# jscanvic/Scale-Equivariant-Imaging

Hardware: AMD Instinct MI355X
Metric: training images/sec (256x256 crops), proposed-loss deblur (higher is better)
Workload: dtype bf16; 1 GPU; BASELINE configs[1]: deblurring Gaussian_R2 noise=5, proposed loss (SURE + scale-EI), 256x256 pairs cropped to 48 in Loss.forward, ConvolutionalModel hidden=32 scales=5; parameters=645063043, batch_per_gpu=32, global_batch=32, parallelism=dp1

## Files before the change

### include/sei_hip.h

```cpp
#ifndef SEI_HIP_H
#define SEI_HIP_H

#include <stddef.h>
#include <stdint.h>

#ifdef __cplusplus
extern "C" {
#endif

#define SEI_OK 0
#define SEI_ERR_BAD_ARG 10001
#define SEI_ERR_TOO_LARGE 10002


#define SEI_ABI_VERSION 12
int sei_abi_version(void);
int sei_build_target(char *name, int n);

int sei_event_create(void **event);
int sei_event_destroy(void *event);
int sei_event_record_external(void *event, void *stream);
int sei_stream_wait_event(void *stream, void *event);

int sei_graph_node_counts(void *graph, int *kernel_nodes, int *all_nodes);
// ... 380 lines not shown
int sei_dwstream_bf16_jobs(const SeiDwStreamJob *jobs, int njobs, void *stream);
size_t sei_dwstream_bf16_eligible(int Mo, int Ni, int ldy, int ldx, long long K1, long long K2);

int sei_rowgemm_bf16(const uint16_t *A, int lda, const uint16_t *W, int ldw, float *D32, int ld32, uint16_t *D16,
                     int ld16, long long M, int N, int K, int nv, int epilogue, const float *bias, const float *R1,
                     const float *R2, int ldr, void *stream);
size_t sei_rowgemm_bf16_eligible(long long M, int N, int K, int epilogue, int out16);

int sei_rowgemm_lnbwd_bf16(const uint16_t *A, int lda, const uint16_t *W, int ldw, long long M, int K, const float *x,
                           const float *gamma, const float *mean, const float *rstd, const float *res, float *gx, int C,
                           float *ggamma, float *gbeta, const float *row_scale, uint16_t *y16, int ldy, float *colsum,
                           float *work, size_t work_floats, void *stream);
size_t sei_rowgemm_lnbwd_bf16_eligible(long long M, int K, int C);
size_t sei_rowgemm_lnbwd_work_floats(int C);

int sei_rowgemm_dgelu_bf16(const uint16_t *A, int lda, const uint16_t *W, int ldw, const uint16_t *A2, int lda2,
                           const uint16_t *W2, int ldw2, const float *bias2, int nv, uint16_t *D16, int ld16, long long M,
                           int N, int K, void *stream);
size_t sei_rowgemm_dgelu_bf16_eligible(long long M, int N, int K);

int sei_rowgemm_ln_bf16(const uint16_t *A, int lda, const uint16_t *W, int ldw, long long M, int K, int C, const float *bias,
                        const float *row_scale, const float *res, float *out, const float *gamma, const float *beta,
                        float eps, int ones_col, uint16_t *h16, int ldh, float *mean, float *rstd, void *stream);
size_t sei_rowgemm_ln_bf16_eligible(long long M, int K, int C);

int sei_rowgemm_gelu_bf16(const uint16_t *A, int lda, const uint16_t *W, int ldw, const float *bias, int nv, uint16_t *D16,
                          int ld16, long long M, int N, int K, int one_at, void *stream);

size_t sei_drunet_work_bytes(int B, int H, int W);
int sei_drunet_conv3x3(const uint16_t *X, const uint16_t *Wt, int Cin, int Cout, int B, int H, int W, int epilogue,
// ... 67 lines not shown
```

### scale-equivariant-imaging_amd/_native.py

```python
import ctypes
import os

import torch

_HERE = os.path.dirname(os.path.abspath(__file__))
LIB_PATH = os.environ.get("SEI_HIP_LIBRARY") or os.path.join(_HERE, "libsei_hip.so")

SEI_REDUCE_BLOCKS = 256

_c = ctypes
_P, _I, _F, _Z, _L = _c.c_void_p, _c.c_int, _c.c_float, _c.c_size_t, _c.c_longlong

SIGNATURES = {
    "sei_abi_version": [],
    "sei_event_create": [_P],
    "sei_event_destroy": [_P],
    "sei_event_record_external": [_P, _P],
    "sei_stream_wait_event": [_P, _P],
    "sei_graph_node_counts": [_P, _P, _P],
    "sei_build_target": [_c.c_char_p, _I],
    "sei_blur_sep_circ": [_P, _P, _P, _P, _I, _I, _I, _I, _I, _I, _P],
    "sei_blur_dense_circ": [_P, _P, _P, _I, _I, _I, _I, _I, _I, _P],
    "sei_blur_dense_pad": [_P, _P, _P, _I, _I, _I, _I, _I, _I, _I, _P, _P],
    "sei_circ_filter_sep": [_P, _P, _P, _P, _I, _I, _I, _P],
# ... 98 lines not shown
    "sei_swin_attn_bwd_bf16": [_P, _P, _P, _P, _P, _P, _P, _I, _I, _I, _I, _I, _F, _P],
    "sei_pad_nhwc": [_P, _P, _I, _I, _I, _I, _I, _P],
    "sei_unpad_nhwc": [_P, _P, _P, _I, _I, _I, _I, _I, _P],
    "sei_rowscale": [_P, _P, _P, _P, _Z, _I, _P],
    "sei_pack": [_P, _P, _P, _Z, _I, _P],
    "sei_unpack_add": [_P, _P, _P, _Z, _P],
    "sei_ln_fwd_bf16_pad": [_P, _P, _P, _P, _P, _P, _Z, _I, _I, _F, _I, _P],
    "sei_ln_bwd_pad": [_P, _P, _P, _P, _P, _P, _P, _P, _P, _Z, _I, _I, _P, _Z, _P],
    "sei_cast_pad_bf16": [_P, _P, _P, _P, _Z, _I, _I, _P, _Z, _P],
    "sei_pad_nhwc_bf16": [_P, _P, _I, _I, _I, _I, _I, _I, _P],
    "sei_pad_nhwc_bf16_ones": [_P, _P, _I, _I, _I, _I, _I, _I, _I, _P],
    "sei_gemm_bf16nt_conv": [_P, _I, _P, _P, _I, _P, _P, _I, _I, _I, _P, _P],
    "sei_gemm_bf16nt_conv_unpad": [_P, _I, _P, _P, _I, _P, _P, _I, _I, _I, _I, _P, _I, _P],
    "sei_rowgemm_bf16": [_P, _I, _P, _I, _P, _I, _P, _I, _L, _I, _I, _I, _I, _P, _P, _P, _I, _P],
    "sei_rowgemm_lnbwd_bf16": [_P, _I, _P, _I, _L, _I, _P, _P, _P, _P, _P, _P, _I, _P, _P, _P, _P, _I, _P, _P, _Z, _P],
    "sei_rowgemm_dgelu_bf16": [_P, _I, _P, _I, _P, _I, _P, _I, _P, _I, _P, _I, _L, _I, _I, _P],
    "sei_rowgemm_ln_bf16": [_P, _I, _P, _I, _L, _I, _I, _P, _P, _P, _P, _P, _P, _F, _I, _P, _I, _P, _P, _P],
    "sei_rowgemm_gelu_bf16": [_P, _I, _P, _I, _P, _I, _P, _I, _L, _I, _I, _I, _P],
    "sei_tokgrad_bf16_blocks": [_P, _I, _L, _L, _P],
    "sei_tokgrad_bf16": [_P, _P, _I, _P, _P, _I, _P, _I, _I, _I, _L, _L, _P],
    "sei_dwstream_bf16_jobs": [_P, _I, _P],
    "sei_adam_fused": [_P, _P, _I, _P, _P, _Z, _F, _F, _F, _F, _F, _I, _F, _P, _P],
    "sei_adam_scalars": [_F, _F, _F, _F, _F, _I, _P, _P],
    "sei_adam_scalars_to_device": [_F, _F, _F, _F, _F, _I, _P, _P],
    "sei_sgd_fused": [_P, _P, _P, _P, _Z, _Z, _F, _F, _P, _P, _I, _P],
    "sei_sgd_penalty_finish": [_P, _Z, _P, _P],
    "sei_adam_anchor_fused": [_P, _P, _P, _P, _P, _P, _Z, _Z, _F, _F, _F, _F, _F, _I, _F, _P, _P, _I, _P],
    "sei_drunet_conv3x3": [_P, _P, _I, _I, _I, _I, _I, _I, _P, _P, _P, _P, _P],
    "sei_drunet_conv3x3_ex": [_P, _P, _I, _I, _I, _I, _I, _I, _P, _P, _P, _P, _I, _P],
    "sei_drunet_down": [_P, _P, _I, _I, _I, _I, _I, _P, _P, _P],
# ... 80 lines not shown
    "sei_dwconv7_bwd_weight_workspace": [_I, _I, _I, _I],
    "sei_dwconv7_bwd_weight_workspace_ex": [_I, _I, _I, _I, _I],
    "sei_ln_bwd_workspace": [_Z, _I],
    "sei_dwconv7_ln_fwd_launches": [_I, _I, _I, _I],
    "sei_sepmap2_bf16_eligible": [_I, _I, _I, _I, _I, _I],
    "sei_sepmap2_bf16_pack_elems": [_I, _I, _I, _I],
    "sei_sepmap2_big_eligible": [_I, _I, _I, _I, _I, _I],
    "sei_sepmap2_big_pack_elems": [_I, _I, _I, _I],
    "sei_sepmap2_big_work_elems": [_I, _I, _I, _I, _I, _I],
    "sei_swin_partials_floats": [_I],
    "sei_tokgrad_bf16_eligible": [_I, _I, _I, _I, _L, _L],
    "sei_dwstream_bf16_eligible": [_I, _I, _I, _I, _L, _L],
    "sei_mlp_fused_eligible": [_L, _I],
    "sei_rowgemm_bf16_eligible": [_L, _I, _I, _I, _I],
    "sei_rowgemm_lnbwd_bf16_eligible": [_L, _I, _I],
    "sei_rowgemm_lnbwd_work_floats": [_I],
    "sei_ln_bwd_part_offset": [_Z, _I],
    "sei_ln_bwd_part_count": [_Z, _I],
    "sei_rowgemm_dgelu_bf16_eligible": [_L, _I, _I],
    "sei_rowgemm_ln_bf16_eligible": [_L, _I, _I],
    "sei_gemm_bf16nt_plan": [_I, _I, _I, _I, _I, _I, _I, _I],
    "sei_gemm_bf16nt_plan_ws": [_I, _I, _I, _I, _I, _I, _I, _I, _Z],
    "sei_gemm_bf16nt_dw2_adam_plan": [_I, _I, _I, _I, _I],
    "sei_gemm_bf16nt_dw2_adam_groupable": [_I, _I, _I, _I],
    "sei_conv3x3_bwd_weight_parts_count": [_I, _I, _I, _I, _I, _I, _I],
    "sei_sepmap2_small_eligible": [_I, _I, _I, _I, _I, _I],
    "sei_cast_bf16_colsum_parts_count": [_I, _I],
    "sei_sgd_partials": [_Z, _Z, _I],
    "sei_adam_anchor_partials": [_Z, _Z, _I],
    "sei_drunet_work_bytes": [_I, _I, _I],
# ... 169 lines not shown
```

### scale-equivariant-imaging_amd/csrc/token_gemm.hip

```cpp
#include "rm_image.h"

namespace {

constexpr int TG_NW = 8, TG_NT = 64 * TG_NW;
constexpr int TG_WCN = 4;
constexpr int TG_RB = 6, TG_CB = 3;
constexpr int TG_NPIECE = 48 / TG_NW;
constexpr int TG_STAGE = 6 * RM_IMG;
constexpr int TG_MAX_BLOCKS = SEI_TOKGRAD_MAX_BLOCKS;

struct TokGradArgs {
    SeiTokGradBlock blk[TG_MAX_BLOCKS];
    int nblk;
    int kt_seg, kt_total;
    int workers_per_xcd;
};

struct TgRange {
    int bsel, kt0, nt;
};
__device__ __forceinline__ TgRange tg_range(const TokGradArgs &g) {
    const int xcd = blockIdx.x & 7, slot = blockIdx.x >> 3;
    const int wslot = slot / g.nblk, bsel = slot - wslot * g.nblk;
    if (wslot >= g.workers_per_xcd) return {0, 0, 0};
// ... 151 lines not shown
    const unsigned short *A2 = nullptr, *W2 = nullptr;
    int lda2 = 0, ldw2 = 0;
    const float *beta2 = nullptr;
    float *mean_out = nullptr, *rstd_out = nullptr;
    float eps = 0.f;
    int ones_col = 0;
    int gelu_one_at = -1;
};

constexpr int RG_EPI_LNBWD = 100;
constexpr int RG_EPI_DGELU2 = 101;
constexpr int RG_EPI_RES_LN = 102;
constexpr int RG_EPI_SCALE_RES_LN = 103;
constexpr int RG_EPI_GELU16 = 104;

template <int KT, int NBT, int TR, int WN, int WR, int EPI, bool OUT16>
__global__ __launch_bounds__(RG_NT, (EPI == RG_EPI_GELU16 ? 4 : 1)) void rowgemm_kernel(RowGemmArgs g) {
    constexpr int WK = 8 / (WN * WR);
    static_assert(WN * WR * WK == 8 && (WK == 1 || WK == 2), "eight waves");
    constexpr int NB = (NBT + WN - 1) / WN;
    constexpr int NBX = NBT % WN;
    constexpr int RB = TR / WR / 16;
    constexpr int KS = 2 * KT / WK;
    static_assert(TR % (16 * WR) == 0 && (2 * KT) % WK == 0, "whole blocks per wave");
    constexpr int NP = 16 * NBT;
    constexpr int LDP = NP + 4;
    constexpr bool TWO = EPI == RG_EPI_DGELU2;
    constexpr int OPS = TWO ? 2 : 1;
    constexpr int STAGE = OPS * KT * TR * 128;
    constexpr int P = KT * TR / 8;
    constexpr int EMAX = (P + 7) / 8;
    constexpr int QR = NP / 4;
    constexpr bool LNB = EPI == RG_EPI_LNBWD;
    constexpr bool LNF = EPI == RG_EPI_RES_LN || EPI == RG_EPI_SCALE_RES_LN;
    constexpr bool LNX = LNB || LNF;
    static_assert(!LNX || (NBT == 12 && TR == 32), "the LayerNorm epilogues own 32 rows x 192 columns: 16 lanes per row");
    constexpr int GQ = (!LNX && (OUT16 || EPI == SEI_EPI_MUL_DGELU || TWO)) ? 2 : 1;
    constexpr bool GELU16 = EPI == RG_EPI_GELU16;
    static_assert(!GELU16 || (OUT16 && WK == 1 && NBX == 0), "bf16 output only; whole column blocks per wave, all of K");
    constexpr bool P16 = ((EPI == SEI_EPI_BIAS || EPI == SEI_EPI_NONE) && OUT16) || TWO || GELU16;
    constexpr int LDP16 = NP + 8;
    static_assert(!P16 || WK == 1, "the bf16 patch has nothing to add up");
    constexpr int IR = QR / GQ;
    constexpr int IPT = (TR * IR + RG_NT - 1) / RG_NT;
    constexpr bool RAGGED = TR * IR % RG_NT != 0;
    constexpr int QPT = IPT * GQ;
    static_assert(TR % 16 == 0 && QR % GQ == 0, "whole items");
    constexpr bool HAS_ROWS = EPI == SEI_EPI_BIAS_RES || EPI == SEI_EPI_BIAS_SCALE_RES || EPI == SEI_EPI_MUL_DGELU;
    constexpr bool HAS_BIAS = EPI == SEI_EPI_BIAS || EPI == SEI_EPI_BIAS_GELU || EPI == SEI_EPI_BIAS_RES ||
                              EPI == SEI_EPI_BIAS_SCALE_RES || LNF;
    constexpr int UNR = IPT > 3 ? (GQ == 2 ? 2 : 3) : IPT;
    constexpr int NAUX = LNF ? 3 + (EPI == RG_EPI_SCALE_RES_LN ? 1 : 0) : LNB ? 8 + (OUT16 ? 1 : 0)
                             : (HAS_ROWS ? QPT : 0) + (EPI == SEI_EPI_BIAS_SCALE_RES ? QPT : 0);
    constexpr int PATCH_ONE = (P16 ? TR * LDP16 * 2 : TR * LDP * 4 + 15) / 16 * 16;
    constexpr int AUX_BYTES = GELU16 ? 0 : (LNF ? 3 : 1) * NP * 4;
    constexpr bool PATCH2 = !GELU16 && 3 * STAGE + 2 * PATCH_ONE + AUX_BYTES <= 160 * 1024;
    __shared__ __attribute__((aligned(1024))) char smem[3 * STAGE + (PATCH2 ? 2 : 1) * PATCH_ONE + AUX_BYTES];
    float *const patch0 = reinterpret_cast<float *>(smem + 3 * STAGE);
    float *lbias = reinterpret_cast<float *>(smem + 3 * STAGE + (PATCH2 ? 2 : 1) * PATCH_ONE);
    float *lgam = lbias + NP, *lbet = lgam + NP;

    const int tid = threadIdx.x, lane = tid & 63;
    const int wave = __builtin_amdgcn_readfirstlane(tid >> 6);
    const int wn = wave % WN, wr = (wave / WN) % WR, wk = wave / (WN * WR);
    const int nbw = (NBX == 0 || wn < NBX) ? NB : NB - 1;
    const int nb0 = (NBX == 0 || wn < NBX) ? NB * wn : NB * NBX + (NB - 1) * (wn - NBX);
    const int l16 = lane & 15, lg = lane >> 4;
    const int G = gridDim.x, b = blockIdx.x;
    if (b >= g.tiles) return;
    const int nt = (g.tiles - b + G - 1) / G;

    bf16x8 wf[NB][KS];
#pragma unroll
    for (int nb = 0; nb < NB; ++nb)
#pragma unroll
        for (int s = 0; s < KS; ++s)
            wf[nb][s] = *reinterpret_cast<const bf16x8 *>(g.W + (size_t)(16 * (nb0 + min(nb, nbw - 1)) + l16) * g.ldw +
                                                          32 * (wk * KS + s) + 8 * lg);
    bf16x8 wf2[TWO ? NB : 1][TWO ? KS : 1];
    float bias2[TWO ? NB : 1];
    if constexpr (TWO) {
#pragma unroll
        for (int nb = 0; nb < NB; ++nb) {
#pragma unroll
            for (int s = 0; s < KS; ++s)
                wf2[nb][s] = *reinterpret_cast<const bf16x8 *>(g.W2 + (size_t)(16 * (nb0 + min(nb, nbw - 1)) + l16) * g.ldw2 +
                                                               32 * (wk * KS + s) + 8 * lg);
            const int c = 16 * (nb0 + min(nb, nbw - 1)) + l16;
            bias2[nb] = c < g.nv ? g.bias[c] : 0.f;
        }
#pragma unroll
// ... 16 lines not shown
#pragma unroll
        for (int nb = 0; nb < NB; ++nb) is_one[nb] = 16 * (nb0 + min(nb, nbw - 1)) + l16 == g.gelu_one_at;
    }
    if constexpr (P16 && (EPI == SEI_EPI_BIAS || GELU16)) {
#pragma unroll
        for (int nb = 0; nb < NB; ++nb) {
            const int c = 16 * (nb0 + min(nb, nbw - 1)) + l16;
            biasr[nb] = c < g.nv ? g.bias[c] : 0.f;
        }
#pragma unroll
        for (int nb = 0; nb < NB; ++nb) asm volatile("" : "+v"(biasr[nb]));
    }
    unsigned offa[EMAX];
#pragma unroll
    for (int e = 0; e < EMAX; ++e) {
        const int q = min(wave + 8 * e, P - 1), im = q / (TR / 8), p = q % (TR / 8);
        const int r = 8 * p + (lane >> 3);
        const int c = (lane & 7) ^ ((r >> 1) & 7);
        offa[e] = (unsigned)r * (unsigned)g.lda * 2u + 128u * im + 16u * c;
    }
    unsigned offa2[TWO ? EMAX : 1];
    if constexpr (TWO) {
#pragma unroll
        for (int e = 0; e < EMAX; ++e) {
            const int q = min(wave + 8 * e, P - 1), im = q / (TR / 8), p = q % (TR / 8);
            const int r = 8 * p + (lane >> 3);
            const int c = (lane & 7) ^ ((r >> 1) & 7);
            offa2[e] = (unsigned)r * (unsigned)g.lda2 * 2u + 128u * im + 16u * c;
        }
    }
// ... 33 lines not shown
            const float *rows = EPI == SEI_EPI_BIAS_SCALE_RES ? g.R2 : g.R1;
#pragma unroll
            for (int i = 0; i < QPT; ++i) {
                const size_t row = (size_t)tile * TR + quad_row(i);
                const int qc = quad_col(i);
                const float *src = rows + row * g.ldr + (qc < g.nv ? qc : 0);
                asm volatile("global_load_dwordx4 %0, %1, off" : "=v"(a[i]) : "v"(src) : "memory");
                if constexpr (EPI == SEI_EPI_BIAS_SCALE_RES) {
                    const float *ssrc = g.R1 + row;
                    asm volatile("global_load_dword %0, %1, off" : "=v"(sc[i]) : "v"(ssrc) : "memory");
                }
            }
        }
    };

    const int er = tid >> 4, el = tid & 15;
    const int nvq = g.nv >> 2;
    f32x4 lx[LNX ? 3 : 1], lr[LNB ? 3 : 1], ag[LNB ? 3 : 1], ab[LNB ? 3 : 1], ac[LNB ? 3 : 1];
    float lmu = 0.f, lrs = 0.f, lsc = 1.f;
    if constexpr (LNF) {
        for (int c = tid; c < NP; c += RG_NT) {
            lgam[c] = c < g.nv ? g.gamma[c] : 0.f;
            lbet[c] = c < g.nv ? g.beta2[c] : 0.f;
        }
    }
    if constexpr (LNB) {
        for (int c = tid; c < NP; c += RG_NT) lbias[c] = c < g.nv ? g.gamma[c] : 0.f;
#pragma unroll
        for (int k = 0; k < 3; ++k) ag[k] = ab[k] = ac[k] = f32x4{0.f, 0.f, 0.f, 0.f};
    }
    auto load_ln = [&](int t) {
        if constexpr (LNF) {
            const int tile = b + min(t, nt - 1) * G;
            const size_t row = (size_t)tile * TR + er;
            const float *rows = EPI == RG_EPI_SCALE_RES_LN ? g.R2 : g.R1;
#pragma unroll
            for (int k = 0; k < 3; ++k) {
                const float *xs = rows + row * g.ldr + 4 * min(el + 16 * k, nvq - 1);
                asm volatile("global_load_dwordx4 %0, %1, off" : "=v"(lx[k]) : "v"(xs) : "memory");
            }
            if constexpr (EPI == RG_EPI_SCALE_RES_LN) {
                const float *cs = g.R1 + row;
                asm volatile("global_load_dword %0, %1, off" : "=v"(lsc) : "v"(cs) : "memory");
            }
        }
        if constexpr (LNB) {
            const int tile = b + min(t, nt - 1) * G;
            const size_t row = (size_t)tile * TR + er;
#pragma unroll
            for (int k = 0; k < 3; ++k) {
                const int c = 4 * min(el + 16 * k, nvq - 1);
                const float *xs = g.R1 + row * g.ldr + c, *rs = g.R2 + row * g.ldr + c;
                asm volatile("global_load_dwordx4 %0, %1, off" : "=v"(lx[k]) : "v"(xs) : "memory");
                asm volatile("global_load_dwordx4 %0, %1, off" : "=v"(lr[k]) : "v"(rs) : "memory");
            }
            const float *ms = g.mean + row, *ss = g.rstd + row;
            asm volatile("global_load_dword %0, %1, off" : "=v"(lmu) : "v"(ms) : "memory");
            asm volatile("global_load_dword %0, %1, off" : "=v"(lrs) : "v"(ss) : "memory");
            if constexpr (OUT16) {
                const float *cs = g.scale + row;
                asm volatile("global_load_dword %0, %1, off" : "=v"(lsc) : "v"(cs) : "memory");
            }
        }
    };

    issue(0);
    issue(1);
    if (P % 8 != 0 && wave < P % 8) sei_wait_vmcnt<NDMA_HI>();
    else sei_wait_vmcnt<NDMA_LO>();
    sei_lds_barrier();

    for (int t = 0; t < nt; ++t) {
        float *const patch = PATCH2 ? reinterpret_cast<float *>(reinterpret_cast<char *>(patch0) + (t & 1) * PATCH_ONE) : patch0;
        load_aux(t, cur, curs);
        load_ln(t);
        __builtin_amdgcn_sched_barrier(0);
// ... 33 lines not shown
                        float v;
                        if constexpr (TWO) v = acc[0][nb][j] * sei_dgelu_bf16out(acc2[nb][j] + bias2[nb]);
                        else v = is_one[nb] ? 1.0f : sei_gelu_bf16out(acc[0][nb][j] + biasr[nb]);
                        const __bf16 h = (__bf16)v;
                        pw16[(16 * rb + j) * LDP16 + 16 * nb] = __builtin_bit_cast(unsigned short, h);
                    }
            }
        } else {
#pragma unroll
        for (int rb = 0; rb < RB; ++rb)
#pragma unroll
            for (int nb = 0; nb < NB; ++nb) acc[rb][nb] = f32x4{0.f, 0.f, 0.f, 0.f};
#pragma unroll
        for (int s = 0; s < KS; ++s) {
            const int sg = wk * KS + s;
            const char *img = st + (sg >> 1) * (TR * 128) + (wr * RB * 16 + l16) * 128 + (((4 * (sg & 1) + lg) ^ (l16 >> 1)) * 16);
#pragma unroll
            for (int rb = 0; rb < RB; ++rb) {
                const bf16x8 fa = *reinterpret_cast<const bf16x8 *>(img + rb * 16 * 128);
#pragma unroll
                for (int nb = 0; nb < NB; ++nb) {
                    if (NBX != 0 && nb == NB - 1 && nbw < NB) break;
                    acc[rb][nb] = __builtin_amdgcn_mfma_f32_16x16x32_bf16(fa, wf[nb][s], acc[rb][nb], 0, 0, 0);
                }
            }
        }
        }
        if (P % 8 != 0 && wave < P % 8) sei_wait_vmcnt<NAUX + NDMA_HI>();
        else sei_wait_vmcnt<NAUX + NDMA_LO>();
        if constexpr (P16 && !GELU16 && !TWO) {
            unsigned short *pw16 = reinterpret_cast<unsigned short *>(patch) + (wr * RB * 16 + 4 * lg) * LDP16 + 16 * nb0 + l16;
#pragma unroll
            for (int rb = 0; rb < RB; ++rb)
#pragma unroll
// ... 94 lines not shown
                } else if (qk == nvq && g.ones_col) {
                    y[0] = 1.0f;
                }
                uint2 h;
                h.x = sei_pack2_bf16(y[0], y[1]);
                h.y = sei_pack2_bf16(y[2], y[3]);
                *reinterpret_cast<uint2 *>(g.D16 + row * g.ld16 + 4 * qk) = h;
            }
        }
        if constexpr (LNB) {
            __builtin_amdgcn_sched_barrier(0);
            if (P % 8 != 0 && wave < P % 8) sei_wait_vmcnt<NDMA_HI>();
            else sei_wait_vmcnt<NDMA_LO>();
            __builtin_amdgcn_sched_barrier(0);
#pragma unroll
            for (int k = 0; k < 3; ++k) {
                asm volatile("" : "+v"(lx[k]));
                asm volatile("" : "+v"(lr[k]));
            }
            asm volatile("" : "+v"(lmu));
            asm volatile("" : "+v"(lrs));
            if constexpr (OUT16) asm volatile("" : "+v"(lsc));
            f32x4 gh[3], xh[3], tq[3];
            float s1 = 0.f, s2 = 0.f;
#pragma unroll
            for (int k = 0; k < 3; ++k) {
                const bool valid = el + 16 * k < nvq;
                gh[k] = *reinterpret_cast<const f32x4 *>(patch + er * LDP + 4 * (el + 16 * k));
                const f32x4 gm = *reinterpret_cast<const f32x4 *>(lbias + 4 * (el + 16 * k));
#pragma unroll
                for (int j = 0; j < 4; ++j) {
                    xh[k][j] = (lx[k][j] - lmu) * lrs;
                    tq[k][j] = gh[k][j] * gm[j];
                }
                if (valid) {
                    s1 += (tq[k][0] + tq[k][1]) + (tq[k][2] + tq[k][3]);
                    s2 += (tq[k][0] * xh[k][0] + tq[k][1] * xh[k][1]) + (tq[k][2] * xh[k][2] + tq[k][3] * xh[k][3]);
                    ag[k] += gh[k] * xh[k];
                    ab[k] += gh[k];
                }
            }
#pragma unroll
            for (int off = 8; off > 0; off >>= 1) {
                s1 += __shfl_xor(s1, off, 16);
                s2 += __shfl_xor(s2, off, 16);
            }
            const float invC = 1.0f / (float)g.nv;
            s1 *= invC;
            s2 *= invC;
            const size_t row = row0 + er;
#pragma unroll
            for (int k = 0; k < 3; ++k) {
                const int qk = el + 16 * k;
                const bool valid = qk < nvq;
                f32x4 o;
#pragma unroll
                for (int j = 0; j < 4; ++j) o[j] = lrs * (tq[k][j] - s1 - xh[k][j] * s2) + lr[k][j];
                if (valid) *reinterpret_cast<f32x4 *>(g.D32 + row * g.ld32 + 4 * qk) = o;
                if constexpr (OUT16) {
                    f32x4 ys;
#pragma unroll
                    for (int j = 0; j < 4; ++j) ys[j] = valid ? o[j] * lsc : 0.f;
                    if constexpr (KT != 9) ac[k] += ys;
                    uint2 h;
                    h.x = sei_pack2_bf16(ys[0], ys[1]);
                    h.y = sei_pack2_bf16(ys[2], ys[3]);
                    *reinterpret_cast<uint2 *>(g.D16 + row * g.ld16 + 4 * qk) = h;
                }
            }
        }
        if constexpr (P16) {
#pragma unroll
            for (int it = 0; it < IPT; ++it) {
                if (RAGGED && it == IPT - 1 && tid + RG_NT * it >= TR * IR) break;
                const int idx = tid + RG_NT * it, qr = idx / IR, qc = 8 * (idx % IR);
                const uint4 h = *reinterpret_cast<const uint4 *>(reinterpret_cast<const unsigned short *>(patch) + qr * LDP16 + qc);
                *reinterpret_cast<uint4 *>(g.D16 + (row0 + qr) * g.ld16 + qc) = h;
            }
        }
#pragma unroll UNR
        for (int it = 0; it < ((LNX || P16) ? 0 : IPT); ++it) {
            if (RAGGED && it == IPT - 1 && tid + RG_NT * it >= TR * IR) break;
            f32x4 v[GQ];
// ... 25 lines not shown
                h.x = sei_pack2_bf16(ge[0], ge[1]);
                h.y = sei_pack2_bf16(ge[2], ge[3]);
                *reinterpret_cast<uint2 *>(g.D16 + row * g.ld16 + qc) = h;
            } else if constexpr (GQ == 2) {
                uint4 h;
                h.x = sei_pack2_bf16(v[0][0], v[0][1]);
                h.y = sei_pack2_bf16(v[0][2], v[0][3]);
                h.z = sei_pack2_bf16(v[GQ - 1][0], v[GQ - 1][1]);
                h.w = sei_pack2_bf16(v[GQ - 1][2], v[GQ - 1][3]);
                *reinterpret_cast<uint4 *>(g.D16 + row * g.ld16 + qc) = h;
            }
        }
        if constexpr (!PATCH2) sei_lds_barrier();
    }
    sei_wait_vmcnt<0>();
    if constexpr (LNB) {
        static_assert(3 * STAGE >= 3 * 32 * 48 * 16, "the ring holds the partial sums");
        __builtin_amdgcn_s_barrier();
        f32x4 *red = reinterpret_cast<f32x4 *>(smem);
#pragma unroll
        for (int k = 0; k < 3; ++k) {
            red[(0 * 32 + er) * 48 + el + 16 * k] = ag[k];
            red[(1 * 32 + er) * 48 + el + 16 * k] = ab[k];
            red[(2 * 32 + er) * 48 + el + 16 * k] = ac[k];
        }
        __syncthreads();
        if (tid < 144) {
            const int sel = tid / 48, qk = tid - sel * 48;
            f32x4 a = f32x4{0.f, 0.f, 0.f, 0.f};
            for (int r = 0; r < 32; ++r) a += red[(sel * 32 + r) * 48 + qk];
            if (qk < nvq) *reinterpret_cast<f32x4 *>(g.part + ((size_t)b * 3 + sel) * g.nv + 4 * qk) = a;
        }
    }
}

template <int KT, int NBT, int TR, int WN, int WR, int EPI, bool OUT16>
int rg_launch(const RowGemmArgs &g, int M, hipStream_t s, int per_cu = 1) {
    RowGemmArgs a = g;
    a.tiles = M / TR;
    const int grid = a.tiles < 256 * per_cu ? a.tiles : 256 * per_cu;
    hipLaunchKernelGGL((rowgemm_kernel<KT, NBT, TR, WN, WR, EPI, OUT16>), dim3((unsigned)grid), dim3(RG_NT), 0, s, a);
    return sei_launch_status();
}

bool rg_operands_ok(const uint16_t *A, int lda, const uint16_t *W, int ldw, int K) {
    return A && W && lda >= K && ldw >= K && lda % 8 == 0 && ldw % 8 == 0 && (((uintptr_t)A | (uintptr_t)W) & 15) == 0 &&
           (unsigned long long)64 * (size_t)lda * 2 < (1ull << 32);
}
int rg_fill_operands(RowGemmArgs &g, const uint16_t *A, int lda, const uint16_t *W, int ldw, long long M, int K) {
    SEI_REQUIRE(M > 0 && M % 64 == 0 && M < (1ll << 31) && rg_operands_ok(A, lda, W, ldw, K));
    g.A = A; g.W = W; g.lda = lda; g.ldw = ldw;
    return SEI_OK;
}

bool tg_block_ok(const SeiTokGradBlock &b, long long K2) {
    if (!b.Y1 || !b.X1 || !b.D || (K2 && (!b.Y2 || !b.X2))) return false;
// ... 127 lines not shown
    if (y16) SEI_REQUIRE(ldy >= 192 && ldy % 4 == 0 && ((uintptr_t)y16 & 7) == 0);
    g.R1 = x; g.R2 = res; g.ldr = C;
    g.D32 = gx; g.D16 = y16; g.ld32 = C; g.ld16 = ldy; g.nv = C;
    g.mean = mean; g.rstd = rstd; g.gamma = gamma; g.scale = row_scale; g.part = work;
    hipStream_t s = (hipStream_t)stream;
    const int m = (int)M, groups = m / 32 < 256 ? m / 32 : 256;
    int rc;
    if (K == 384)
        rc = y16 ? rg_launch<6, 12, 32, 4, 1, RG_EPI_LNBWD, true>(g, m, s) : rg_launch<6, 12, 32, 4, 1, RG_EPI_LNBWD, false>(g, m, s);
    else
        rc = y16 ? rg_launch<9, 12, 32, 4, 1, RG_EPI_LNBWD, true>(g, m, s) : rg_launch<9, 12, 32, 4, 1, RG_EPI_LNBWD, false>(g, m, s);
    if (rc != 0 || !ggamma) return rc;
    return sei_fold_now(sei_fold_job(SEI_FOLD_SPLIT, work, groups, 3 * C, C, ggamma, gbeta, colsum), s);
}

extern "C" size_t sei_rowgemm_dgelu_bf16_eligible(long long M, int N, int K) {
    return (M > 0 && M % 64 == 0 && M < (1ll << 31) && N == 384 && K == 192) ? 1 : 0;
}

extern "C" int sei_rowgemm_dgelu_bf16(const uint16_t *A, int lda, const uint16_t *W, int ldw, const uint16_t *A2, int lda2,
                                      const uint16_t *W2, int ldw2, const float *bias2, int nv, uint16_t *D16, int ld16,
                                      long long M, int N, int K, void *stream) {
    RowGemmArgs g;
    SEI_REQUIRE(bias2 && D16 && sei_rowgemm_dgelu_bf16_eligible(M, N, K));
    SEI_REQUIRE(rg_fill_operands(g, A, lda, W, ldw, M, K) == SEI_OK && rg_operands_ok(A2, lda2, W2, ldw2, K));
    SEI_REQUIRE(((uintptr_t)D16 & 15) == 0 && nv > 0 && nv <= N && ld16 >= N && ld16 % 8 == 0);
    g.A2 = A2; g.W2 = W2; g.lda2 = lda2; g.ldw2 = ldw2;
    g.bias = bias2; g.D16 = D16; g.ld16 = ld16; g.nv = nv;
    return rg_launch<3, 24, 32, 8, 1, RG_EPI_DGELU2, true>(g, (int)M, (hipStream_t)stream);
}
// ... 38 lines not shown
```

### scale-equivariant-imaging_amd/models/_ops.py

```python
import os

import torch

import _native as N
from . import _mats, _wgrad
from ._gemm import (EPI_ACCUM, EPI_BIAS, EPI_BIAS_GELU, EPI_BIAS_RES, EPI_BIAS_ROWSCALE, EPI_MUL_DGELU, EPI_NONE,
                    SPLITK_COUNTER_BYTES, SPLITK_WS_MIB, SPLITK_WS_STREAMS, _SPLITK_WS, _gemm_call, _in_forward_mode,
                    compute_dtype_scope, gemm, gemm_mixed, gemm_nt16, gemm_x3, get_compute_dtype, joint_rows,
                    own_splitk_workspace, profile_gemms, release_splitk_workspace, reset_splitk_counters, set_compute_dtype,
                    splitk_workspace)
from ._joint import JointCtx, _NotJoint, joint_ctx, walk_backward
from ._shadow import (ShadowState, _new_plain_state, _transposed16, _transposed16_cached, plain_shadow_is_current,
                      refresh_plain_shadow, set_stale_masters, shadow, split_x2, weights_updated)
from ._wgrad import (_state_for, begin_step, colsum16_into, defer_fold, direct_bf16_launches, flush_weight_grads,
                     fused_adam_launches, merged_weight_grads, note_forward, register_gradient_range,
                     set_direct_bf16_grads, set_fused_adam, set_weight_grad_merging, set_weight_grad_milestone, state_of,
                     weight_grad16, weight_grad16_group, weight_grad_views)

LN_EPS = 1e-6


def grad_of(p):
    if p.grad is None:
        view = getattr(p, "_sei_grad_view", None)
# ... 231 lines not shown
    B, H, W, C = x.shape
    M = B * H * W
    gh = resample(gu.view(B, ctx.hw[2], ctx.hw[3], C), ctx.mats_t, H, W).view(M, C)
    res = None if gskip is None else gskip.contiguous().view(M, C)
    gx = layer_norm_bwd(x.view(M, C), gamma, mean, rstd, gh, grad_of(gamma), grad_of(beta), res=res).view(B, H, W, C)
    return (gx if ctx.needs_input_grad[0] else None), None, None, None, None, None, None


def _check_skip(skip, shape):
    skip = _nhwc(skip)
    if tuple(skip.shape) != shape:
        raise ValueError("skip connection shape mismatch")
    return skip


def _upsample_tail(ctx, go, gh, resample):
    u, mean, rstd = ctx.saved_tensors[:3]
    gamma, beta = ctx.params[:2]
    gu = layer_norm_bwd(u.view(-1, u.shape[-1]), gamma, mean, rstd, gh, grad_of(gamma), grad_of(beta))
    gx = None
    if ctx.needs_input_grad[0]:
        gx = resample(gu.view(u.shape), ctx.mats_t, *ctx.in_hw)
    gskip = go if ctx.needs_input_grad[1] else None
    return gx, gskip, None, None, None, None, None


class DownsampleFn(torch.autograd.Function):

    @staticmethod
    def forward(ctx, x, gamma, beta, w, b, rate, with_skip=False):
        _no_joint_form()
        ctx.dtype = get_compute_dtype()
        ctx.set_materialize_grads(False)
        x = _nhwc(x)
# ... 255 lines not shown
        else:
            gemm_nt16(h, w16, M, Co, C, EPI_BIAS, out32=out, bias=b)
        ctx.save_for_backward(u, mean, rstd, h)
        ctx.params, ctx.mats_t, ctx.in_hw = (gamma, beta, w, b), bwd, (H, W)
        return out.view(B, Ho, Wo, Co)

    @_in_forward_mode
    def backward(ctx, go):
        u, mean, rstd, h = ctx.saved_tensors
        gamma, beta, w, b = ctx.params
        B, Ho, Wo, C = u.shape
        M, Co = B * Ho * Wo, w.shape[0]
        go = go.contiguous()
        go2 = go.view(M, Co)
        go16 = cast16(go2, colsum_into_=grad_of(b))
        gh = torch.empty((M, C), dtype=torch.float32, device=u.device)
        gemm_nt16(go16, shadow(w), M, C, Co, EPI_NONE, out32=gh, b_rmajor=True)
        weight_grad16(go16, h, grad_of(w).view(Co, C))
        return _upsample_tail(ctx, go, gh, sepmap2_16)

    @staticmethod
    def joint_ctx(c1, c2, rec):
        return JointCtx(c1, [rec.joint(a, b) for a, b in zip(c1.saved_tensors, c2.saved_tensors)])

    @staticmethod
    def walk(ctx, g, skips):
        gx, gskip = UpsampleFn16.backward(ctx, g)[:2]
        skips.append(gskip)
        return gx


class Conv3x3Fn(torch.autograd.Function):
    @staticmethod
    def forward(ctx, x, w, b, res, nchw_in, nchw_out):
# ... 49 lines not shown
```

### scale-equivariant-imaging_amd/models/_wgrad.py

```python
import collections
import os
import weakref

import torch

import _native as N
from . import _gemm
from ._gemm import EPI_ACCUM, EPI_NONE, _gemm_call, gemm_mixed, gemm_nt16

TOKEN_STREAMING = os.environ.get("SEI_SWIN_TILED") != "1"

DWSTREAM = os.environ.get("SEI_NO_DWSTREAM") != "1"

DEFERRED_FOLDS = os.environ.get("SEI_NO_DEFERRED_FOLDS") != "1"

SINK_ADAM, SINK_BF16 = "adam", "direct16"
_SINKS = {SINK_ADAM: ("sei_gemm_bf16nt_dw2_adam", "fused optimizer step"),
          SINK_BF16: ("sei_gemm_bf16nt_dw2_bf16out", "bf16 gradients written into the exchange buffer")}

ADAM_GROUP = os.environ.get("SEI_NO_ADAM_GROUP") != "1"

_Queued = collections.namedtuple("_Queued", "job operands grad flops")
_QueuedAdam = collections.namedtuple("_QueuedAdam", "job operands hyper flops args")


def _segments(pairs):
    (g1, x1), (g2, x2) = pairs[0], pairs[-1]
    return g1, x1, g2, x2, g1.shape[0], (g2.shape[0] if len(pairs) == 2 else 0)


def colsum16_into(acc, x16):
    M, Nn = x16.shape
    N.call("sei_colsum_bf16", x16.data_ptr(), acc.data_ptr(), M, Nn)


# ... 410 lines not shown
```

Measured before the change: 2730 images/s.

## Fuse upsample data-gradient GEMM with LayerNorm backward epilogue

In the bf16 upsample backward, the data-gradient GEMM (go16 x W) is fused with the LayerNorm backward in a new row-GEMM variant. The variant reads the weight transposed, supports a 32-wide K image and runs without a residual. The fusion removes the float32 gh intermediate and its round trip through global memory, plus a separate LayerNorm-backward launch. The price is more template complexity (multi-pass row ownership, strided transposed weight loads) and a new reduction path for the gamma/beta partials, which could be slower than the tuned original.

```diff
diff --git a/include/sei_hip.h b/include/sei_hip.h
--- a/include/sei_hip.h
+++ b/include/sei_hip.h
@@ -418,6 +418,11 @@
 size_t sei_rowgemm_lnbwd_bf16_eligible(long long M, int K, int C);
 size_t sei_rowgemm_lnbwd_work_floats(int C);
 
+int sei_rowgemm_lnbwd_rm_bf16(const uint16_t *A, int lda, const uint16_t *W, int ldw, long long M, int K, const float *x,
+                              const float *gamma, const float *mean, const float *rstd, const float *res, float *gx,
+                              int C, float *ggamma, float *gbeta, float *work, size_t work_floats, void *stream);
+size_t sei_rowgemm_lnbwd_rm_bf16_eligible(long long M, int K, int C);
+
 int sei_rowgemm_dgelu_bf16(const uint16_t *A, int lda, const uint16_t *W, int ldw, const uint16_t *A2, int lda2,
                            const uint16_t *W2, int ldw2, const float *bias2, int nv, uint16_t *D16, int ld16, long long M,
                            int N, int K, void *stream);
diff --git a/scale-equivariant-imaging_amd/_native.py b/scale-equivariant-imaging_amd/_native.py
--- a/scale-equivariant-imaging_amd/_native.py
+++ b/scale-equivariant-imaging_amd/_native.py
@@ -136,6 +136,7 @@
     "sei_gemm_bf16nt_conv_unpad": [_P, _I, _P, _P, _I, _P, _P, _I, _I, _I, _I, _P, _I, _P],
     "sei_rowgemm_bf16": [_P, _I, _P, _I, _P, _I, _P, _I, _L, _I, _I, _I, _I, _P, _P, _P, _I, _P],
     "sei_rowgemm_lnbwd_bf16": [_P, _I, _P, _I, _L, _I, _P, _P, _P, _P, _P, _P, _I, _P, _P, _P, _P, _I, _P, _P, _Z, _P],
+    "sei_rowgemm_lnbwd_rm_bf16": [_P, _I, _P, _I, _L, _I, _P, _P, _P, _P, _P, _P, _I, _P, _P, _P, _Z, _P],
     "sei_rowgemm_dgelu_bf16": [_P, _I, _P, _I, _P, _I, _P, _I, _P, _I, _P, _I, _L, _I, _I, _P],
     "sei_rowgemm_ln_bf16": [_P, _I, _P, _I, _L, _I, _I, _P, _P, _P, _P, _P, _P, _F, _I, _P, _I, _P, _P, _P],
     "sei_rowgemm_gelu_bf16": [_P, _I, _P, _I, _P, _I, _P, _I, _L, _I, _I, _I, _P],
@@ -246,6 +247,7 @@
     "sei_mlp_fused_eligible": [_L, _I],
     "sei_rowgemm_bf16_eligible": [_L, _I, _I, _I, _I],
     "sei_rowgemm_lnbwd_bf16_eligible": [_L, _I, _I],
+    "sei_rowgemm_lnbwd_rm_bf16_eligible": [_L, _I, _I],
     "sei_rowgemm_lnbwd_work_floats": [_I],
     "sei_ln_bwd_part_offset": [_Z, _I],
     "sei_ln_bwd_part_count": [_Z, _I],
diff --git a/scale-equivariant-imaging_amd/csrc/token_gemm.hip b/scale-equivariant-imaging_amd/csrc/token_gemm.hip
--- a/scale-equivariant-imaging_amd/csrc/token_gemm.hip
+++ b/scale-equivariant-imaging_amd/csrc/token_gemm.hip
@@ -189,27 +189,35 @@
 constexpr int RG_EPI_SCALE_RES_LN = 103;
 constexpr int RG_EPI_GELU16 = 104;
 
-template <int KT, int NBT, int TR, int WN, int WR, int EPI, bool OUT16>
+template <int KT, int NBT, int TR, int WN, int WR, int EPI, bool OUT16, bool RES = true, int KW = 64, bool WT = false>
 __global__ __launch_bounds__(RG_NT, (EPI == RG_EPI_GELU16 ? 4 : 1)) void rowgemm_kernel(RowGemmArgs g) {
     constexpr int WK = 8 / (WN * WR);
+    static_assert(KW == 64 || (KW == 32 && KT == 1 && EPI == RG_EPI_LNBWD), "a 32-wide image: K = 32, one k-step");
+    constexpr int IMG_ROW = 2 * KW;
     static_assert(WN * WR * WK == 8 && (WK == 1 || WK == 2), "eight waves");
     constexpr int NB = (NBT + WN - 1) / WN;
     constexpr int NBX = NBT % WN;
     constexpr int RB = TR / WR / 16;
-    constexpr int KS = 2 * KT / WK;
-    static_assert(TR % (16 * WR) == 0 && (2 * KT) % WK == 0, "whole blocks per wave");
+    constexpr int KS = KT * (KW / 32) / WK;
+    static_assert(TR % (16 * WR) == 0 && (KT * (KW / 32)) % WK == 0, "whole blocks per wave");
     constexpr int NP = 16 * NBT;
     constexpr int LDP = NP + 4;
     constexpr bool TWO = EPI == RG_EPI_DGELU2;
     constexpr int OPS = TWO ? 2 : 1;
-    constexpr int STAGE = OPS * KT * TR * 128;
-    constexpr int P = KT * TR / 8;
+    constexpr int STAGE = OPS * KT * TR * IMG_ROW;
+    constexpr int P = KT * TR * IMG_ROW / 1024;
     constexpr int EMAX = (P + 7) / 8;
     constexpr int QR = NP / 4;
     constexpr bool LNB = EPI == RG_EPI_LNBWD;
     constexpr bool LNF = EPI == RG_EPI_RES_LN || EPI == RG_EPI_SCALE_RES_LN;
     constexpr bool LNX = LNB || LNF;
-    static_assert(!LNX || (NBT == 12 && TR == 32), "the LayerNorm epilogues own 32 rows x 192 columns: 16 lanes per row");
+    static_assert(!LNF || (NBT == 12 && TR == 32), "the LayerNorm epilogue owns 32 rows x 192 columns: 16 lanes per row");
+    static_assert(!LNB || (TR == 32 && (NBT == 12 || NBT == 8 || NBT == 32)), "the LayerNorm backward owns 32 whole rows");
+    constexpr int LPR = (LNB && NBT == 32) ? 32 : 16, LPR_SH = LPR == 32 ? 5 : 4;
+    constexpr int NQ = LNX ? (NP / 4) / LPR : 1, RPP = RG_NT / LPR, PASSES = LNX ? TR / RPP : 1;
+    static_assert(!LNX || (NQ * LPR * 4 == NP && PASSES * RPP == TR), "whole rows per pass");
+    static_assert(!LNF || (NQ == 3 && PASSES == 1), "as before");
+    static_assert(RES || (LNB && !OUT16), "only the float32 LayerNorm backward may go without a residual");
     constexpr int GQ = (!LNX && (OUT16 || EPI == SEI_EPI_MUL_DGELU || TWO)) ? 2 : 1;
     constexpr bool GELU16 = EPI == RG_EPI_GELU16;
     static_assert(!GELU16 || (OUT16 && WK == 1 && NBX == 0), "bf16 output only; whole column blocks per wave, all of K");
@@ -225,7 +233,7 @@
     constexpr bool HAS_BIAS = EPI == SEI_EPI_BIAS || EPI == SEI_EPI_BIAS_GELU || EPI == SEI_EPI_BIAS_RES ||
                               EPI == SEI_EPI_BIAS_SCALE_RES || LNF;
     constexpr int UNR = IPT > 3 ? (GQ == 2 ? 2 : 3) : IPT;
-    constexpr int NAUX = LNF ? 3 + (EPI == RG_EPI_SCALE_RES_LN ? 1 : 0) : LNB ? 8 + (OUT16 ? 1 : 0)
+    constexpr int NAUX = LNF ? 3 + (EPI == RG_EPI_SCALE_RES_LN ? 1 : 0) : LNB ? PASSES * ((RES ? 2 : 1) * NQ + 2) + (OUT16 ? 1 : 0)
                              : (HAS_ROWS ? QPT : 0) + (EPI == SEI_EPI_BIAS_SCALE_RES ? QPT : 0);
     constexpr int PATCH_ONE = (P16 ? TR * LDP16 * 2 : TR * LDP * 4 + 15) / 16 * 16;
     constexpr int AUX_BYTES = GELU16 ? 0 : (LNF ? 3 : 1) * NP * 4;
@@ -250,6 +258,16 @@
     for (int nb = 0; nb < NB; ++nb)
 #pragma unroll
         for (int s = 0; s < KS; ++s)
+            if constexpr (WT) {
+                unsigned short wv[8];
+#pragma unroll
+                for (int j = 0; j < 8; ++j)
+                    wv[j] = g.W[(size_t)(32 * (wk * KS + s) + 8 * lg + j) * g.ldw + 16 * (nb0 + min(nb, nbw - 1)) + l16];
+                u32x4 wp;
+#pragma unroll
+                for (int j = 0; j < 4; ++j) wp[j] = (unsigned)wv[2 * j] | ((unsigned)wv[2 * j + 1] << 16);
+                wf[nb][s] = __builtin_bit_cast(bf16x8, wp);
+            } else
             wf[nb][s] = *reinterpret_cast<const bf16x8 *>(g.W + (size_t)(16 * (nb0 + min(nb, nbw - 1)) + l16) * g.ldw +
                                                           32 * (wk * KS + s) + 8 * lg);
     bf16x8 wf2[TWO ? NB : 1][TWO ? KS : 1];
@@ -296,6 +314,13 @@
     unsigned offa[EMAX];
 #pragma unroll
     for (int e = 0; e < EMAX; ++e) {
+        if constexpr (KW == 32) {
+            const int q = min(wave + 8 * e, P - 1), im = q / (TR / 16), p = q % (TR / 16);
+            const int r = 16 * p + (lane >> 2);
+            const int c = (lane & 3) ^ ((0 - (r >> 2)) & 3);
+            offa[e] = (unsigned)r * (unsigned)g.lda * 2u + 64u * im + 16u * c;
+            continue;
+        }
         const int q = min(wave + 8 * e, P - 1), im = q / (TR / 8), p = q % (TR / 8);
         const int r = 8 * p + (lane >> 3);
         const int c = (lane & 7) ^ ((r >> 1) & 7);
@@ -359,10 +384,12 @@
         }
     };
 
-    const int er = tid >> 4, el = tid & 15;
+    const int er = tid >> LPR_SH, el = tid & (LPR - 1);
     const int nvq = g.nv >> 2;
-    f32x4 lx[LNX ? 3 : 1], lr[LNB ? 3 : 1], ag[LNB ? 3 : 1], ab[LNB ? 3 : 1], ac[LNB ? 3 : 1];
-    float lmu = 0.f, lrs = 0.f, lsc = 1.f;
+    f32x4 lx[PASSES * NQ], lr[(LNB && RES) ? PASSES * NQ : 1], ag[NQ], ab[NQ], ac[NQ];
+    float lmu[PASSES], lrs[PASSES], lsc = 1.f;
+#pragma unroll
+    for (int p = 0; p < PASSES; ++p) lmu[p] = lrs[p] = 0.f;
     if constexpr (LNF) {
         for (int c = tid; c < NP; c += RG_NT) {
             lgam[c] = c < g.nv ? g.gamma[c] : 0.f;
@@ -372,7 +399,7 @@
     if constexpr (LNB) {
         for (int c = tid; c < NP; c += RG_NT) lbias[c] = c < g.nv ? g.gamma[c] : 0.f;
 #pragma unroll
-        for (int k = 0; k < 3; ++k) ag[k] = ab[k] = ac[k] = f32x4{0.f, 0.f, 0.f, 0.f};
+        for (int k = 0; k < NQ; ++k) ag[k] = ab[k] = ac[k] = f32x4{0.f, 0.f, 0.f, 0.f};
     }
     auto load_ln = [&](int t) {
         if constexpr (LNF) {
@@ -391,20 +418,24 @@
         }
         if constexpr (LNB) {
             const int tile = b + min(t, nt - 1) * G;
-            const size_t row = (size_t)tile * TR + er;
-#pragma unroll
-            for (int k = 0; k < 3; ++k) {
-                const int c = 4 * min(el + 16 * k, nvq - 1);
-                const float *xs = g.R1 + row * g.ldr + c, *rs = g.R2 + row * g.ldr + c;
-                asm volatile("global_load_dwordx4 %0, %1, off" : "=v"(lx[k]) : "v"(xs) : "memory");
-                asm volatile("global_load_dwordx4 %0, %1, off" : "=v"(lr[k]) : "v"(rs) : "memory");
-            }
-            const float *ms = g.mean + row, *ss = g.rstd + row;
-            asm volatile("global_load_dword %0, %1, off" : "=v"(lmu) : "v"(ms) : "memory");
-            asm volatile("global_load_dword %0, %1, off" : "=v"(lrs) : "v"(ss) : "memory");
-            if constexpr (OUT16) {
-                const float *cs = g.scale + row;
-                asm volatile("global_load_dword %0, %1, off" : "=v"(lsc) : "v"(cs) : "memory");
+#pragma unroll
+            for (int p = 0; p < PASSES; ++p) {
+                const size_t row = (size_t)tile * TR + RPP * p + er;
+#pragma unroll
+                for (int k = 0; k < NQ; ++k) {
+                    const int c = 4 * min(el + LPR * k, nvq - 1);
+                    const float *xs = g.R1 + row * g.ldr + c, *rs = RES ? g.R2 + row * g.ldr + c : nullptr;
+                    asm volatile("global_load_dwordx4 %0, %1, off" : "=v"(lx[NQ * p + k]) : "v"(xs) : "memory");
+                    if constexpr (RES) asm volatile("global_load_dwordx4 %0, %1, off" : "=v"(lr[NQ * p + k]) : "v"(rs) : "memory");
+                }
+                const float *ms = g.mean + row, *ss = g.rstd + row;
+                asm volatile("global_load_dword %0, %1, off" : "=v"(lmu[p]) : "v"(ms) : "memory");
+                asm volatile("global_load_dword %0, %1, off" : "=v"(lrs[p]) : "v"(ss) : "memory");
+                if constexpr (OUT16) {
+                    static_assert(!OUT16 || PASSES == 1, "one row factor per thread");
+                    const float *cs = g.scale + row;
+                    asm volatile("global_load_dword %0, %1, off" : "=v"(lsc) : "v"(cs) : "memory");
+                }
             }
         }
     };
@@ -468,10 +499,11 @@
 #pragma unroll
         for (int s = 0; s < KS; ++s) {
             const int sg = wk * KS + s;
-            const char *img = st + (sg >> 1) * (TR * 128) + (wr * RB * 16 + l16) * 128 + (((4 * (sg & 1) + lg) ^ (l16 >> 1)) * 16);
+            const char *img = KW == 32 ? st + sg * (TR * 64) + (wr * RB * 16 + l16) * 64 + ((lg ^ ((0 - (l16 >> 2)) & 3)) * 16)
+                                       : st + (sg >> 1) * (TR * 128) + (wr * RB * 16 + l16) * 128 + (((4 * (sg & 1) + lg) ^ (l16 >> 1)) * 16);
 #pragma unroll
             for (int rb = 0; rb < RB; ++rb) {
-                const bf16x8 fa = *reinterpret_cast<const bf16x8 *>(img + rb * 16 * 128);
+                const bf16x8 fa = *reinterpret_cast<const bf16x8 *>(img + rb * 16 * IMG_ROW);
 #pragma unroll
                 for (int nb = 0; nb < NB; ++nb) {
                     if (NBX != 0 && nb == NB - 1 && nbw < NB) break;
@@ -596,23 +628,29 @@
             else sei_wait_vmcnt<NDMA_LO>();
             __builtin_amdgcn_sched_barrier(0);
 #pragma unroll
-            for (int k = 0; k < 3; ++k) {
+            for (int k = 0; k < PASSES * NQ; ++k) {
                 asm volatile("" : "+v"(lx[k]));
-                asm volatile("" : "+v"(lr[k]));
-            }
-            asm volatile("" : "+v"(lmu));
-            asm volatile("" : "+v"(lrs));
+                if constexpr (RES) asm volatile("" : "+v"(lr[k]));
+            }
+#pragma unroll
+            for (int p = 0; p < PASSES; ++p) {
+                asm volatile("" : "+v"(lmu[p]));
+                asm volatile("" : "+v"(lrs[p]));
+            }
             if constexpr (OUT16) asm volatile("" : "+v"(lsc));
-            f32x4 gh[3], xh[3], tq[3];
+#pragma unroll
+            for (int p = 0; p < PASSES; ++p) {
+            const int pr = RPP * p + er;
+            f32x4 gh[NQ], xh[NQ], tq[NQ];
             float s1 = 0.f, s2 = 0.f;
 #pragma unroll
-            for (int k = 0; k < 3; ++k) {
-                const bool valid = el + 16 * k < nvq;
-                gh[k] = *reinterpret_cast<const f32x4 *>(patch + er * LDP + 4 * (el + 16 * k));
-                const f32x4 gm = *reinterpret_cast<const f32x4 *>(lbias + 4 * (el + 16 * k));
+            for (int k = 0; k < NQ; ++k) {
+                const bool valid = el + LPR * k < nvq;
+                gh[k] = *reinterpret_cast<const f32x4 *>(patch + pr * LDP + 4 * (el + LPR * k));
+                const f32x4 gm = *reinterpret_cast<const f32x4 *>(lbias + 4 * (el + LPR * k));
 #pragma unroll
                 for (int j = 0; j < 4; ++j) {
-                    xh[k][j] = (lx[k][j] - lmu) * lrs;
+                    xh[k][j] = (lx[NQ * p + k][j] - lmu[p]) * lrs[p];
                     tq[k][j] = gh[k][j] * gm[j];
                 }
                 if (valid) {
@@ -623,21 +661,24 @@
                 }
             }
 #pragma unroll
-            for (int off = 8; off > 0; off >>= 1) {
-                s1 += __shfl_xor(s1, off, 16);
-                s2 += __shfl_xor(s2, off, 16);
+            for (int off = LPR / 2; off > 0; off >>= 1) {
+                s1 += __shfl_xor(s1, off, LPR);
+                s2 += __shfl_xor(s2, off, LPR);
             }
             const float invC = 1.0f / (float)g.nv;
             s1 *= invC;
             s2 *= invC;
-            const size_t row = row0 + er;
-#pragma unroll
-            for (int k = 0; k < 3; ++k) {
-                const int qk = el + 16 * k;
+            const size_t row = row0 + pr;
+#pragma unroll
+            for (int k = 0; k < NQ; ++k) {
+                const int qk = el + LPR * k;
                 const bool valid = qk < nvq;
                 f32x4 o;
 #pragma unroll
-                for (int j = 0; j < 4; ++j) o[j] = lrs * (tq[k][j] - s1 - xh[k][j] * s2) + lr[k][j];
+                for (int j = 0; j < 4; ++j) {
+                    o[j] = lrs[p] * (tq[k][j] - s1 - xh[k][j] * s2);
+                    if constexpr (RES) o[j] += lr[NQ * p + k][j];
+                }
                 if (valid) *reinterpret_cast<f32x4 *>(g.D32 + row * g.ld32 + 4 * qk) = o;
                 if constexpr (OUT16) {
                     f32x4 ys;
@@ -649,6 +690,7 @@
                     h.y = sei_pack2_bf16(ys[2], ys[3]);
                     *reinterpret_cast<uint2 *>(g.D16 + row * g.ld16 + 4 * qk) = h;
                 }
+            }
             }
         }
         if constexpr (P16) {
@@ -704,7 +746,7 @@
         if constexpr (!PATCH2) sei_lds_barrier();
     }
     sei_wait_vmcnt<0>();
-    if constexpr (LNB) {
+    if constexpr (LNB && NQ == 3 && PASSES == 1) {
         static_assert(3 * STAGE >= 3 * 32 * 48 * 16, "the ring holds the partial sums");
         __builtin_amdgcn_s_barrier();
         f32x4 *red = reinterpret_cast<f32x4 *>(smem);
@@ -721,15 +763,37 @@
             for (int r = 0; r < 32; ++r) a += red[(sel * 32 + r) * 48 + qk];
             if (qk < nvq) *reinterpret_cast<f32x4 *>(g.part + ((size_t)b * 3 + sel) * g.nv + 4 * qk) = a;
         }
-    }
-}
-
-template <int KT, int NBT, int TR, int WN, int WR, int EPI, bool OUT16>
+    } else if constexpr (LNB) {
+        static_assert(RPP >= 8, "eight chains");
+        static_assert(!OUT16 && sizeof(smem) >= (size_t)RPP * QR * 16, "the LDS holds one partial sum");
+        f32x4 *red = reinterpret_cast<f32x4 *>(smem);
+#pragma unroll
+        for (int sel = 0; sel < 2; ++sel) {
+            __syncthreads();
+#pragma unroll
+            for (int k = 0; k < NQ; ++k) red[er * QR + el + LPR * k] = sel == 0 ? ag[k] : ab[k];
+            __syncthreads();
+            if (tid < QR) {
+                f32x4 a[8];
+#pragma unroll
+                for (int c = 0; c < 8; ++c) a[c] = red[c * QR + tid];
+#pragma unroll
+                for (int r = 8; r < RPP; ++r) a[r & 7] += red[r * QR + tid];
+                const f32x4 s = ((a[0] + a[1]) + (a[2] + a[3])) + ((a[4] + a[5]) + (a[6] + a[7]));
+                if (tid < nvq) *reinterpret_cast<f32x4 *>(g.part + ((size_t)b * 3 + sel) * g.nv + 4 * tid) = s;
+            }
+        }
+        if (tid < QR && tid < nvq)
+            *reinterpret_cast<f32x4 *>(g.part + ((size_t)b * 3 + 2) * g.nv + 4 * tid) = f32x4{0.f, 0.f, 0.f, 0.f};
+    }
+}
+
+template <int KT, int NBT, int TR, int WN, int WR, int EPI, bool OUT16, bool RES = true, int KW = 64, bool WT = false>
 int rg_launch(const RowGemmArgs &g, int M, hipStream_t s, int per_cu = 1) {
     RowGemmArgs a = g;
     a.tiles = M / TR;
     const int grid = a.tiles < 256 * per_cu ? a.tiles : 256 * per_cu;
-    hipLaunchKernelGGL((rowgemm_kernel<KT, NBT, TR, WN, WR, EPI, OUT16>), dim3((unsigned)grid), dim3(RG_NT), 0, s, a);
+    hipLaunchKernelGGL((rowgemm_kernel<KT, NBT, TR, WN, WR, EPI, OUT16, RES, KW, WT>), dim3((unsigned)grid), dim3(RG_NT), 0, s, a);
     return sei_launch_status();
 }
 
@@ -887,6 +951,37 @@
     return sei_fold_now(sei_fold_job(SEI_FOLD_SPLIT, work, groups, 3 * C, C, ggamma, gbeta, colsum), s);
 }
 
+extern "C" size_t sei_rowgemm_lnbwd_rm_bf16_eligible(long long M, int K, int C) {
+    return (M > 0 && M % 64 == 0 && M < (1ll << 31) && ((K == 32 && C == 128) || (K == 128 && C == 512))) ? 1 : 0;
+}
+
+extern "C" int sei_rowgemm_lnbwd_rm_bf16(const uint16_t *A, int lda, const uint16_t *W, int ldw, long long M, int K,
+                                         const float *x, const float *gamma, const float *mean, const float *rstd,
+                                         const float *res, float *gx, int C, float *ggamma, float *gbeta, float *work,
+                                         size_t work_floats, void *stream) {
+    RowGemmArgs g;
+    SEI_REQUIRE(A && W && x && gamma && mean && rstd && gx && work && (ggamma != nullptr) == (gbeta != nullptr));
+    SEI_REQUIRE(sei_rowgemm_lnbwd_rm_bf16_eligible(M, K, C) && work_floats >= sei_rowgemm_lnbwd_work_floats(C));
+    SEI_REQUIRE(lda >= K && lda % 8 == 0 && ldw >= C && ((uintptr_t)A & 15) == 0 &&
+                (unsigned long long)32 * (size_t)lda * 2 < (1ull << 32));
+    SEI_REQUIRE((((uintptr_t)x | (uintptr_t)res | (uintptr_t)gx | (uintptr_t)work) & 15) == 0);
+    g.A = A; g.W = W; g.lda = lda; g.ldw = ldw;
+    g.R1 = x; g.R2 = res; g.ldr = C;
+    g.D32 = gx; g.ld32 = C; g.nv = C;
+    g.mean = mean; g.rstd = rstd; g.gamma = gamma; g.part = work;
+    hipStream_t s = (hipStream_t)stream;
+    const int m = (int)M, groups = m / 32 < 256 ? m / 32 : 256;
+    int rc;
+    if (K == 32)
+        rc = res ? rg_launch<1, 8, 32, 4, 2, RG_EPI_LNBWD, false, true, 32, true>(g, m, s)
+                 : rg_launch<1, 8, 32, 4, 2, RG_EPI_LNBWD, false, false, 32, true>(g, m, s);
+    else
+        rc = res ? rg_launch<2, 32, 32, 8, 1, RG_EPI_LNBWD, false, true, 64, true>(g, m, s)
+                 : rg_launch<2, 32, 32, 8, 1, RG_EPI_LNBWD, false, false, 64, true>(g, m, s);
+    if (rc != 0 || !ggamma) return rc;
+    return sei_fold_now(sei_fold_job(SEI_FOLD_SPLIT, work, groups, 3 * C, C, ggamma, gbeta, nullptr), s);
+}
+
 extern "C" size_t sei_rowgemm_dgelu_bf16_eligible(long long M, int N, int K) {
     return (M > 0 && M % 64 == 0 && M < (1ll << 31) && N == 384 && K == 192) ? 1 : 0;
 }
diff --git a/scale-equivariant-imaging_amd/models/_ops.py b/scale-equivariant-imaging_amd/models/_ops.py
--- a/scale-equivariant-imaging_amd/models/_ops.py
+++ b/scale-equivariant-imaging_amd/models/_ops.py
@@ -269,10 +269,25 @@
     return skip
 
 
-def _upsample_tail(ctx, go, gh, resample):
+def _upsample_dgrad_lnbwd(go16, w16, u2d, gamma, beta, mean, rstd):
+    M, C = u2d.shape
+    Co = w16.shape[0]
+    gu = torch.empty_like(u2d)
+    ggamma, gbeta = grad_of(gamma), grad_of(beta)
+    work = torch.empty(N.lib().sei_rowgemm_lnbwd_work_floats(C), dtype=torch.float32, device=u2d.device)
+    deferred = defer_fold(ggamma, gbeta, None, 3 * C, C, N.FOLD_SPLIT, work, 0, min(M // 32, 256))
+    _gemm_call(2.0 * M * C * Co, "sei_rowgemm_lnbwd_rm_bf16", go16.data_ptr(), go16.shape[1], w16.data_ptr(), C, M, Co,
+               u2d.data_ptr(), gamma.data_ptr(), mean.data_ptr(), rstd.data_ptr(), None, gu.data_ptr(), C,
+               None if deferred else ggamma.data_ptr(), None if deferred else gbeta.data_ptr(), work.data_ptr(),
+               work.numel())
+    return gu
+
+
+def _upsample_tail(ctx, go, gh, resample, gu=None):
     u, mean, rstd = ctx.saved_tensors[:3]
     gamma, beta = ctx.params[:2]
-    gu = layer_norm_bwd(u.view(-1, u.shape[-1]), gamma, mean, rstd, gh, grad_of(gamma), grad_of(beta))
+    if gu is None:
+        gu = layer_norm_bwd(u.view(-1, u.shape[-1]), gamma, mean, rstd, gh, grad_of(gamma), grad_of(beta))
     gx = None
     if ctx.needs_input_grad[0]:
         gx = resample(gu.view(u.shape), ctx.mats_t, *ctx.in_hw)
@@ -558,10 +573,15 @@
         go = go.contiguous()
         go2 = go.view(M, Co)
         go16 = cast16(go2, colsum_into_=grad_of(b))
-        gh = torch.empty((M, C), dtype=torch.float32, device=u.device)
-        gemm_nt16(go16, shadow(w), M, C, Co, EPI_NONE, out32=gh, b_rmajor=True)
+        if _wgrad.UPSAMPLE_LNBWD and N.lib().sei_rowgemm_lnbwd_rm_bf16_eligible(M, Co, C):
+            gu = _upsample_dgrad_lnbwd(go16, shadow(w), u.view(M, C), gamma, beta, mean, rstd)
+            gh = None
+        else:
+            gu = None
+            gh = torch.empty((M, C), dtype=torch.float32, device=u.device)
+            gemm_nt16(go16, shadow(w), M, C, Co, EPI_NONE, out32=gh, b_rmajor=True)
         weight_grad16(go16, h, grad_of(w).view(Co, C))
-        return _upsample_tail(ctx, go, gh, sepmap2_16)
+        return _upsample_tail(ctx, go, gh, sepmap2_16, gu=gu)
 
     @staticmethod
     def joint_ctx(c1, c2, rec):
diff --git a/scale-equivariant-imaging_amd/models/_wgrad.py b/scale-equivariant-imaging_amd/models/_wgrad.py
--- a/scale-equivariant-imaging_amd/models/_wgrad.py
+++ b/scale-equivariant-imaging_amd/models/_wgrad.py
@@ -19,6 +19,8 @@
           SINK_BF16: ("sei_gemm_bf16nt_dw2_bf16out", "bf16 gradients written into the exchange buffer")}
 
 ADAM_GROUP = os.environ.get("SEI_NO_ADAM_GROUP") != "1"
+
+UPSAMPLE_LNBWD = os.environ.get("SEI_NO_UPSAMPLE_LNBWD") != "1"
 
 _Queued = collections.namedtuple("_Queued", "job operands grad flops")
 _QueuedAdam = collections.namedtuple("_QueuedAdam", "job operands hyper flops args")
```

Result: no change. 2753 images/s, median of 6 (+0.8%).
